# chngdickson/ov2slam

Measured on AMD Instinct MI355X. Metric: tracked_frames_per_sec, higher is better.
Workload: dtype u8/s16 fixed-point + f32

## Files before the change

include/ov2slam_hip.h:

```cpp
#ifndef OV2SLAM_HIP_H
#define OV2SLAM_HIP_H

#include <stddef.h>
#include <stdint.h>

#ifdef __cplusplus
extern "C" {
#endif

typedef int ov2_status;
enum {
    OV2_OK = 0,
    OV2_ERR_INVALID = -1,
    OV2_ERR_HIP = -2,
    OV2_ERR_NOMEM = -3,
    OV2_ERR_NODEVICE = -4,
    OV2_ERR_UNSUPPORTED = -5
};

typedef struct ov2_ctx ov2_ctx;
typedef struct ov2_images ov2_images;
typedef struct ov2_pyr ov2_pyr;

ov2_status ov2_ctx_create(int device, ov2_ctx **out);
// ... 42 lines not shown
void ov2_pyr_release(ov2_pyr *p);
void ov2_pyr_release_from(ov2_ctx *user, ov2_pyr *p);
int ov2_pyr_batch(const ov2_pyr *p);
int ov2_pyr_nlevels(const ov2_pyr *p);
ov2_status ov2_pyr_level_size(const ov2_pyr *p, int level, int *w, int *h, int *pad);
ov2_status ov2_pyr_download_level(ov2_ctx *ctx, const ov2_pyr *p, int b, int level, uint8_t *img, int16_t *grad);

ov2_status ov2_klt_track_fb(ov2_ctx *ctx, const ov2_pyr *prev, const ov2_pyr *cur, int win, int nlevels,
                            int max_iter, float eps, float err_th, float fb_th, int n, const float *kps_xy,
                            float *priors_xy, uint8_t *status);
ov2_status ov2_klt_track_fb_dev(ov2_ctx *ctx, const ov2_pyr *prev, const ov2_pyr *cur, int win, int nlevels,
                                int max_iter, float eps, float err_th, float fb_th, int n, const float *d_kps_xy,
                                float *d_priors_xy, uint8_t *d_status, const int32_t *d_img_idx,
                                uint32_t *d_iters);

ov2_status ov2_klt_tracking_frame_dev(ov2_ctx *ctx, const ov2_pyr *prev, const ov2_pyr *cur, int win,
                                      int nlevels_full, int max_iter, float eps, float err_th, float fb_th, int n,
                                      const float *d_kps_xy, const float *d_prior_xy, const uint8_t *d_has_prior,
                                      const int32_t *d_img_idx, float *d_out_xy, uint8_t *d_out_status,
                                      int32_t *d_p3p_req , uint32_t *d_iters );

ov2_status ov2_klt_set_lanes(ov2_ctx *ctx, int lanes);
ov2_status ov2_klt_set_stereo_split(ov2_ctx *ctx, int k);

ov2_status ov2_line_min_sad(ov2_ctx *ctx, const ov2_pyr *left, const ov2_pyr *right, int level, int nwinsize, int go_left,
                            int n, const float *pts_xy, float *xprior, float *l1err);
ov2_status ov2_line_min_sad_dev(ov2_ctx *ctx, const ov2_pyr *left, const ov2_pyr *right, int level, int nwinsize,
                                int go_left, int n, const float *d_pts_xy, const int32_t *d_img_idx, float *d_xprior,
                                float *d_l1err);

typedef struct ov2_cam_model {
    double K[4];
    int32_t model;
    int32_t n_coeffs;
    double D[5];
} ov2_cam_model;

ov2_status ov2_stereo_matching(ov2_ctx *ctx, const ov2_pyr *left, const ov2_pyr *right, int win, int nlevels_full,
                               int max_iter, float eps, float err_th, float fb_th, int n, const float *kps_xy,
                               const float *prior_xy, const uint8_t *has_prior, const float *lunpx_xy, int rectified,
                               const double *F_rl, const ov2_cam_model *right_cam, float *out_rxy, uint8_t *out_status);
ov2_status ov2_stereo_matching_dev(ov2_ctx *ctx, const ov2_pyr *left, const ov2_pyr *right, int win, int nlevels_full,
                                   int max_iter, float eps, float err_th, float fb_th, int n, const float *d_kps_xy,
                                   const float *d_prior_xy, const uint8_t *d_has_prior, const int32_t *d_img_idx,
                                   const float *d_lunpx_xy, int rectified, const double *F_rl, const ov2_cam_model *right_cam,
                                   float *d_out_rxy, uint8_t *d_out_status, uint32_t *d_iters);
// ... 414 lines not shown
```

ov2slam_amd/_lib.py:

```python
import ctypes as C
import os

_HERE = os.path.dirname(os.path.abspath(__file__))
LIB_PATH = os.environ.get("OV2SLAM_HIP_LIB") or os.path.join(_HERE, "lib", "libov2hip.so")

vp = C.c_void_p
vpp = C.POINTER(C.c_void_p)
ip = C.POINTER(C.c_int)
fp = C.POINTER(C.c_float)

SIGNATURES = {
    "ov2_ctx_create": (C.c_int, [C.c_int, vpp]),
    "ov2_ctx_create_ex": (C.c_int, [C.c_int, C.c_int, vpp]),
    "ov2_ctx_destroy": (None, [vp]),
    "ov2_last_error": (C.c_char_p, [vp]),
    "ov2_status_string": (C.c_char_p, [C.c_int]),
    "ov2_ctx_synchronize": (C.c_int, [vp]),
    "ov2_ctx_set_kf_overlap": (C.c_int, [vp, C.c_int]),
    "ov2_ctx_set_wave_prio": (C.c_int, [vp, C.c_int]),
    "ov2_ctx_get_wave_prio": (C.c_int, [vp]),
    "ov2_ctx_create_cu": (C.c_int, [C.c_int, C.c_int, C.c_int, C.c_int, vpp]),
    "ov2_ctx_get_cu_share": (C.c_int, [vp]),
    "ov2_ctx_get_cu_mask": (C.c_int, [vp, C.c_int, C.POINTER(C.c_uint32)]),
    "ov2_cu_mask_build": (C.c_int, [C.c_int, C.c_int, C.c_int, C.POINTER(C.c_uint32)]),
# ... 12 lines not shown
    "ov2_memcpy_d2h": (C.c_int, [vp, vp, vp, C.c_size_t]),
    "ov2_memcpy_d2d": (C.c_int, [vp, vp, vp, C.c_size_t]),
    "ov2_images_create": (C.c_int, [vp, C.c_int, C.c_int, C.c_int, vpp]),
    "ov2_images_upload": (C.c_int, [vp, vp, C.c_int, vp, C.c_int]),
    "ov2_images_destroy": (None, [vp]),
    "ov2_pyramid_build": (C.c_int, [vp, vp, C.c_int, C.c_int, C.c_int, C.c_int, C.c_int, C.c_int, C.c_float,
                                    C.c_int, C.c_int, vpp]),
    "ov2_pyramid_build_images": (C.c_int, [vp, vp, C.c_int, C.c_int, C.c_int, C.c_float, C.c_int, C.c_int, vpp]),
    "ov2_pyr_retain": (None, [vp]),
    "ov2_pyr_release": (None, [vp]),
    "ov2_pyr_release_from": (None, [vp, vp]),
    "ov2_pyr_batch": (C.c_int, [vp]),
    "ov2_pyr_nlevels": (C.c_int, [vp]),
    "ov2_pyr_level_size": (C.c_int, [vp, C.c_int, ip, ip, ip]),
    "ov2_pyr_download_level": (C.c_int, [vp, vp, C.c_int, C.c_int, vp, vp]),
    "ov2_klt_track_fb": (C.c_int, [vp, vp, vp, C.c_int, C.c_int, C.c_int, C.c_float, C.c_float, C.c_float,
                                   C.c_int, vp, vp, vp]),
    "ov2_klt_track_fb_dev": (C.c_int, [vp, vp, vp, C.c_int, C.c_int, C.c_int, C.c_float, C.c_float, C.c_float,
                                       C.c_int, vp, vp, vp, vp, vp]),
    "ov2_klt_tracking_frame_dev": (C.c_int, [vp, vp, vp, C.c_int, C.c_int, C.c_int, C.c_float, C.c_float,
                                             C.c_float, C.c_int, vp, vp, vp, vp, vp, vp, vp, vp]),
    "ov2_klt_set_lanes": (C.c_int, [vp, C.c_int]),
    "ov2_klt_set_stereo_split": (C.c_int, [vp, C.c_int]),
    "ov2_line_min_sad": (C.c_int, [vp, vp, vp, C.c_int, C.c_int, C.c_int, C.c_int, vp, vp, vp]),
    "ov2_line_min_sad_dev": (C.c_int, [vp, vp, vp, C.c_int, C.c_int, C.c_int, C.c_int, vp, vp, vp, vp]),
    "ov2_stereo_matching": (C.c_int, [vp, vp, vp, C.c_int, C.c_int, C.c_int, C.c_float, C.c_float, C.c_float, C.c_int,
                                      vp, vp, vp, vp, C.c_int, vp, vp, vp, vp]),
    "ov2_stereo_matching_dev": (C.c_int, [vp, vp, vp, C.c_int, C.c_int, C.c_int, C.c_float, C.c_float, C.c_float, C.c_int,
                                          vp, vp, vp, vp, vp, C.c_int, vp, vp, vp, vp, vp]),
    "ov2_detect_grid": (C.c_int, [vp, vp, C.c_int, C.c_int, C.c_int, C.POINTER(C.c_double), C.c_int, vp, vp, C.c_int, ip, vp]),
    "ov2_detect_grid_batch": (C.c_int, [vp, vp, C.c_int, C.c_int, C.POINTER(C.c_double), ip, vp, vp, C.c_int, ip, vp, C.c_int]),
    "ov2_detect_grid_batch_dev": (C.c_int, [vp, vp, C.c_int, C.c_int, vp, C.c_int, vp, vp, vp, vp, C.c_int, vp, vp, C.c_int]),
    "ov2_fast_detect_batch": (C.c_int, [vp, vp, C.c_int, C.c_int, vp, vp, C.c_int, C.c_int, vp, vp, vp, vp]),
    "ov2_fast_detect_batch_dev": (C.c_int, [vp, vp, C.c_int, C.c_int, C.c_int, vp, vp, C.c_int, C.c_int, vp, vp, vp, vp]),
    "ov2_ba_default_options": (None, [vp, C.c_float]),
    "ov2_ba_solve": (C.c_int, [vp, vp, vp, vp]),
    "ov2_ba_solve_batch": (C.c_int, [vp, C.c_int, vp, vp, vp]),
    "ov2_ba_solve_batch_dev": (C.c_int, [vp, C.c_int, vp, vp, vp]),
    "ov2_pnp_solve_batch_dev": (C.c_int, [vp, C.c_int, vp, vp, vp, vp, vp, vp, C.c_int, C.c_float, C.c_int, C.c_int,
                                          vp, vp, vp, vp]),
    "ov2_map_create": (C.c_int, [vp, C.c_int, C.c_int, C.c_int, vp]),
    "ov2_map_destroy": (None, [vp]),
    "ov2_map_add_keyframe": (C.c_int, [vp, C.c_int, vp, C.c_int, vp, vp, vp, vp, vp]),
    "ov2_map_set_landmarks": (C.c_int, [vp, C.c_int, vp, vp, vp]),
    "ov2_map_set_poses": (C.c_int, [vp, C.c_int, vp, vp]),
    "ov2_map_remove_obs": (C.c_int, [vp, C.c_int, vp, vp]),
# ... 87 lines not shown
```

ov2slam_amd/csrc/ctx.hip:

```cpp
#include "ov2_internal.h"

#include <cstdlib>

ov2_status ov2_set_err(ov2_ctx *ctx, ov2_status s, const char *fmt, ...)
{
    char buf[512];
    va_list ap;
    va_start(ap, fmt);
    vsnprintf(buf, sizeof(buf), fmt, ap);
    va_end(ap);
    if (ctx) {
        std::lock_guard<std::mutex> g(ctx->mu);
        ctx->err = buf;
    }
    return s;
}

extern "C" const char *ov2_status_string(ov2_status s)
{
    switch (s) {
    case OV2_OK: return "ok";
    case OV2_ERR_INVALID: return "invalid argument";
    case OV2_ERR_HIP: return "HIP runtime error";
    case OV2_ERR_NOMEM: return "out of memory";
// ... 91 lines not shown
    if (device < 0 || device >= ndev) return OV2_ERR_INVALID;
    if (hipSetDevice(device) != hipSuccess) return OV2_ERR_HIP;
    uint32_t mask[MAX_MASK_WORDS];
    int mask_words = 0, effective_cus = 0;
    if (n_cus > 0) {
        const int total = device_cus(device);
        if (n_cus >= total || total > 32 * MAX_MASK_WORDS || ov2_cu_mask_build(total, n_cus, layout, mask) != OV2_OK) return OV2_ERR_INVALID;
        mask_words = (total + 31) / 32;
        for (int x = 0; x < OV2_CU_MASK_XCDS; ++x) {
            int bits = 0, own = 0;
            for (int k = x; k < total; k += OV2_CU_MASK_XCDS, ++own) bits += (int)(mask[k >> 5] >> (k & 31) & 1u);
            effective_cus += bits ? bits : own;
        }
    }
    ov2_ctx *c = new ov2_ctx();
    c->device = device;
    c->scratch_dev = nullptr;
    c->scratch_bytes = 0;
    c->tmp_img = nullptr;
    c->ktime_on = false;
    c->wave_prio = high_priority ? OV2_WAVE_PRIO_HIGH : 0;
    c->klt_lanes = 0;
    c->klt_stereo_split = -1;
    c->knn_lanes = 0;
    c->knn_cus = effective_cus;
    c->cu_share = n_cus;
    c->cu_layout = layout;
    c->counts_as_high = false;
    c->lcd_splits = 0;
    c->lcd_calls = 0;
    c->ba_arena = nullptr;
    c->ba_arena_cap = 0;
    c->ba_host = nullptr;
    c->ba_host_cap = 0;
    c->ba_copy_stream = nullptr;
    c->klt_counts[0] = c->klt_counts[1] = nullptr;
    c->klt_counts_words = 0;
    c->klt_counts_cur = 0;
    c->klt_counts_dirty = true;
    c->ba_copy_ev[0] = c->ba_copy_ev[1] = nullptr;
    c->ba_arena2 = nullptr;
    c->ba_arena2_cap = 0;
    c->stage_host = c->stage_dev = nullptr;
    c->stage_cap = 0;
    c->stage_ev = nullptr;
    c->stage_ev_pending = false;
// ... 455 lines not shown
```

ov2slam_amd/csrc/klt.hip:

```cpp
#include <cstdlib>

#include "ov2_internal.h"
#include "ov2_wave.h"

using namespace ov2wave;

namespace {

struct klt_params {
    int win, nlevels, max_iter;
    int wave_prio;
    double eps2;
    float err_th;
    double fb_th;
    float min_eig_thr;
    int rule33;
};

#define W_BITS 14

__device__ __forceinline__ void lk_weights(float a, float b, int &w00, int &w01, int &w10, int &w11)
{
    w00 = (int)__builtin_rintf((1.f - a) * (1.f - b) * (float)(1 << W_BITS));
    w01 = (int)__builtin_rintf(a * (1.f - b) * (float)(1 << W_BITS));
// ... 403 lines not shown
    const unsigned o = J.img_o + (unsigned)(rr0 * J.istride + cc0);
#pragma unroll
    for (int t = 0; t < klt3::NLD; ++t) {
        unsigned a;
        if (klt3::RBYTES == 48) a = o + (unsigned)(t * J.istride + 16 * c);
        else {
            const int sg = min(3 * t + c, 2 * klt3::RROWS - 1);
            a = o + (unsigned)((sg >> 1) * J.istride + (sg & 1) * 16);
        }
        S.v[t] = ld_b128(J.base + (size_t)a);
    }
}
__device__ __forceinline__ void klt3_store_region(const klt3_segs &S, int c, bool store, unsigned char *lj)
{
    if (store) {
#pragma unroll
        for (int t = 0; t < klt3::NLD; ++t) {
            if (klt3::RBYTES == 48) *reinterpret_cast<uint4 *>(lj + t * klt3::RBYTES + 16 * c) = S.v[t];
            else if (3 * t + c < 2 * klt3::RROWS) *reinterpret_cast<uint4 *>(lj + (3 * t + c) * 16) = S.v[t];
        }
    }
}

template <int WIN>
__device__ __forceinline__ int lk_level3(const level_ptrs &I, const level_ptrs &J, int pad, int level, int max_level,
                                         bool run, float kx, float ky, float &nx_io, float &ny_io, int &status,
                                         float &err, const klt_params &P, int c, bool lane_ok, unsigned &passes,
                                         unsigned char *lj)
{
    static_assert(WIN == 9, "three lanes x three columns");
    constexpr int NPX = 3 * WIN, NQ = (NPX + 1) / 2;
    const float FLT_SCALE = 1.f / (float)(1 << 20);
    const float half = (float)(WIN - 1) * 0.5f;
    const float lscale = __builtin_ldexpf(1.f, -level);
    float px = kx * lscale, py = ky * lscale;
    float nx, ny;
    if (level == max_level) { nx = nx_io * lscale; ny = ny_io * lscale; }
    else { nx = nx_io * 2.f; ny = ny_io * 2.f; }
    if (run) { nx_io = nx; ny_io = ny; }

    px -= half; py -= half;
    const int ipx = (int)floorf(px), ipy = (int)floorf(py);
    if (run && (ipx < -WIN || ipx >= I.w || ipy < -WIN || ipy >= I.h)) {
        if (level == 0) { status = 0; err = 0.f; }
        run = false;
    }
    if (!__any(run)) return 0;
    if (run) passes += 1u;
    int w00, w01, w10, w11;
    lk_weights(px - (float)ipx, py - (float)ipy, w00, w01, w10, w11);

// ... 170 lines not shown
            }
        }
        float b1, b2;
        if (__all((unsigned)(pb1 + (1 << 27)) < (1u << 28) && (unsigned)(pb2 + (1 << 27)) < (1u << 28))) {
            b1 = (float)sum3_i32(pb1, c) * FLT_SCALE;
            b2 = (float)sum3_i32(pb2, c) * FLT_SCALE;
        } else {
            b1 = (float)sum3_f64((double)pb1, c) * FLT_SCALE;
            b2 = (float)sum3_f64((double)pb2, c) * FLT_SCALE;
        }
        const float dx = (A12 * b2 - A22 * b1) * D;
        const float dy = (A12 * b1 - A11 * b2) * D;
        if (run) {
            ++iters;
            nx += dx; ny += dy;
            nx_io = nx + half; ny_io = ny + half;
            if ((double)dx * dx + (double)dy * dy <= P.eps2) run = false;
            else if (j > 0 && fabsf(dx + pdx) <= 0.01f && fabsf(dy + pdy) <= 0.01f) {
                nx_io -= dx * 0.5f; ny_io -= dy * 0.5f;
                run = false;
            }
            pdx = dx; pdy = dy;
        }
    }
    return iters;
}

template <int WIN, int GL>
__device__ __forceinline__ int lk_pass(const level_ptrs &I, const level_ptrs &J, int pad, int level, int max_level, bool run,
                                       float kx, float ky, float &nx_io, float &ny_io, int &status, float &err,
                                       const klt_params &P, int sub, bool lane_ok, unsigned &passes, unsigned char *smem, int slot)
{
    if constexpr (GL == 3) {
        return lk_level3<WIN>(I, J, pad, level, max_level, run, kx, ky, nx_io, ny_io, status, err, P, sub, lane_ok, passes,
                              smem + slot * klt3::RSZ);
    } else {
        constexpr int KPW = 64 / GL, WB = klt_lds<WIN>::WB, GB = klt_lds<WIN>::GB;
        return lk_level<WIN, GL>(I, J, pad, level, max_level, run, kx, ky, nx_io, ny_io, status, err, P, sub, passes,
                                 smem + slot * WB, smem + KPW * WB + slot * WB, smem + 2 * KPW * WB + slot * GB);
    }
}

struct __attribute__((aligned(16))) klt_handover { float fx, fy, err; unsigned work; };

template <int WIN, int GL>
__device__ __forceinline__ int fb_track(const ov2_pyr_view &pv, const ov2_pyr_view &cv, int b, bool act, float kx,
                                          float ky, float &fx, float &fy, const klt_params &P, int nlevels, int sub,
                                          bool lane_ok, unsigned &work, unsigned char *smem, int slot,
                                          int l_hi, int l_lo, float err0, unsigned work0, float &err_out)
{
    int status = 1;
    float err = err0;
    unsigned it = work0 & 0xffffu, passes = work0 >> 16;
    for (int l = l_hi; l >= l_lo; --l) {
        const level_ptrs I = level_of(pv, l, b), J = level_of(cv, l, b);
        it += lk_pass<WIN, GL>(I, J, pv.pad, l, nlevels, act, kx, ky, fx, fy, status, err, P, sub, lane_ok, passes, smem, slot);
    }
    if (l_lo > 0) {
        work = it | (passes << 16);
        err_out = err;
        return 0;
    }
    const int W0 = cv.lv[0].w, H0 = cv.lv[0].h;
    int ok = act && status && !(err > P.err_th) &&
             (1.f <= fx && fx < (float)W0 - 1.f && 1.f <= fy && fy < (float)H0 - 1.f);
    int st2 = 1;
    float e2 = 0.f, bx = kx, by = ky;
    {
        const level_ptrs I = level_of(cv, 0, b), J = level_of(pv, 0, b);
        it += lk_pass<WIN, GL>(I, J, cv.pad, 0, 0, ok != 0, fx, fy, bx, by, st2, e2, P, sub, lane_ok, passes, smem, slot);
    }
    if (ok) {
        if (!st2) ok = 0;
        else {
            const float dx = kx - bx, dy = ky - by;
            const double nrm = __dsqrt_rn((double)dx * dx + (double)dy * dy);
            if (nrm > P.fb_th) ok = 0;
        }
    }
    work = it | (passes << 16);
    return ok;
}

template <int WIN, int GL>
__device__ __forceinline__ int fb_track(const ov2_pyr_view &pv, const ov2_pyr_view &cv, int b, bool act, float kx,
                                          float ky, float &fx, float &fy, const klt_params &P, int nlevels, int sub,
                                          bool lane_ok, unsigned &work, unsigned char *smem, int slot)
{
    float err;
    return fb_track<WIN, GL>(pv, cv, b, act, kx, ky, fx, fy, P, nlevels, sub, lane_ok, work, smem, slot, nlevels, 0, 0.f, 0u, err);
}

#define KLT_GL8_MIN_KPS 65536
// ... 101 lines not shown
    const bool retry = mine && is_a && !ok;
    const unsigned long long rm = __ballot(retry);
    if (rm) {
        const int lane = (int)threadIdx.x, leader = __ffsll((long long)rm) - 1;
        int base = 0;
        if (lane == leader) base = (int)atomicAdd(&cnt[2], (unsigned)__popcll(rm));
        base = __shfl(base, leader);
        if (retry) list_c[base + __popcll(rm & ((1ull << lane) - 1ull))] = i;
    }
}

template <int WIN, int KLT_GL, bool SPLIT>
__global__ __launch_bounds__(64) __attribute__((amdgpu_waves_per_eu(KLT_WAVES(WIN, KLT_GL)))) void klt_stage1_kernel(ov2_pyr_view pv, ov2_pyr_view cv, klt_params P, int n,
                                                        const float2 *__restrict__ kps,
                                                        const float2 *__restrict__ prior,
                                                        const int *__restrict__ img_idx, float2 *__restrict__ out_xy,
                                                        unsigned char *__restrict__ out_status,
                                                        unsigned *__restrict__ counts ,
                                                        unsigned *__restrict__ iters, const int *__restrict__ list_a,
                                                        const int *__restrict__ list_b, unsigned *__restrict__ cnt,
                                                        int *__restrict__ list_c,
                                                        int b_word ,
                                                        int split_k ,
                                                        klt_handover *__restrict__ hand )
{
    __shared__ __attribute__((aligned(16))) unsigned char smem[klt_smem<WIN, KLT_GL>::BYTES];
    using M = klt_map<KLT_GL>;
    constexpr int KLT_KPW = M::KPW;
    const int total_a = (int)cnt[0], total_b = (int)cnt[b_word];
    const int groups_b = (total_b + KLT_KPW - 1) / KLT_KPW;
    const bool is_a = (int)blockIdx.x >= groups_b;
    const int g = is_a ? (int)blockIdx.x - groups_b : (int)blockIdx.x;
    const int total = is_a ? total_a : total_b;
    if (g * KLT_KPW >= total) return;
    ov2wave::set_wave_prio(P.wave_prio);
    const int slot = M::slot((int)threadIdx.x), sub = M::sub((int)threadIdx.x), idx = g * KLT_KPW + slot;
    const bool lane_ok = M::lane_ok((int)threadIdx.x);
    const bool act = idx < total && lane_ok;
    const int i = (is_a ? list_a : list_b)[idx < total ? idx : total - 1];
    const float2 kp = kps[i];
    const int b = img_idx ? img_idx[i] : 0;
    float2 pr = (is_a || !P.rule33) ? prior[i] : kp;
    unsigned work = 0;
    const int nl = is_a ? min(1, pv.nlevels - 1) : P.nlevels;
    const bool upper = SPLIT && !is_a;
    float err;
    const int ok = fb_track<WIN, KLT_GL>(pv, cv, b, act, kp.x, kp.y, pr.x, pr.y, P, nl, sub, lane_ok, work, smem, slot, nl,
                                         upper ? split_k + 1 : 0, 0.f, 0u, err);
    if (upper) {
        if (act && sub == 0) hand[i] = klt_handover{pr.x, pr.y, err, work};
        return;
    }
    klt_stage1_finish(act && sub == 0, is_a, i, b, n, ok, pr, work, out_xy, out_status, counts, iters, cnt, list_c);
}

template <int WIN, int KLT_GL>
__global__ __launch_bounds__(64) __attribute__((amdgpu_waves_per_eu(KLT_WAVES(WIN, KLT_GL)))) void klt_stage2_kernel(ov2_pyr_view pv, ov2_pyr_view cv, klt_params P, int n,
                                                        const float2 *__restrict__ kps,
                                                        const int *__restrict__ img_idx, float2 *__restrict__ out_xy,
                                                        unsigned char *__restrict__ out_status,
                                                        const unsigned *__restrict__ counts, int *__restrict__ p3p_req,
                                                        unsigned *__restrict__ iters, const int *__restrict__ list_c,
                                                        const unsigned *__restrict__ cnt, int batch,
                                                        unsigned *__restrict__ next_counts, int next_words,
                                                        const int *__restrict__ list_b, int b_word,
                                                        const float2 *__restrict__ prior,
                                                        int split_k ,
                                                        const klt_handover *__restrict__ hand)
{
    __shared__ __attribute__((aligned(16))) unsigned char smem[klt_smem<WIN, KLT_GL>::BYTES];
    using M = klt_map<KLT_GL>;
    constexpr int KLT_KPW = M::KPW;
    const int slot = M::slot((int)threadIdx.x), sub = M::sub((int)threadIdx.x);
    const bool lane_ok = M::lane_ok((int)threadIdx.x);
    for (int q = blockIdx.x * 64 + threadIdx.x; q < next_words; q += gridDim.x * 64) next_counts[q] = 0u;
    auto tally = [&](int b, int &n3, int &good) {
        n3 = 0; good = 0;
        if constexpr (KLT_GL == 3) {
            for (int q = sub; q < 64; q += 3) {
                const unsigned cw = counts[64 * b + q];
                n3 += (int)(cw & 0xffffu); good += (int)(cw >> 16);
            }
            n3 = sum3_i32(n3, sub); good = sum3_i32(good, sub);
        } else {
            for (int q = 0; q < 64 / KLT_GL; ++q) {
                const unsigned cw = counts[64 * b + sub * (64 / KLT_GL) + q];
                n3 += (int)(cw & 0xffffu); good += (int)(cw >> 16);
            }
            n3 = row_sum_i32<KLT_GL>(n3); good = row_sum_i32<KLT_GL>(good);
        }
    };
// ... 19 lines not shown
    const int i = (is_b ? list_b : list_c)[idx < total ? idx : total - 1];
    const int b = img_idx ? img_idx[i] : 0;
    const float2 kp = kps[i];
    float2 pr;
    int l_hi = P.nlevels;
    float err0 = 0.f;
    unsigned work0 = 0;
    if (is_b) {
        if (split_k >= 0) {
            const klt_handover hr = hand[i];
            pr = make_float2(hr.fx, hr.fy);
            err0 = hr.err; work0 = hr.work; l_hi = split_k;
        } else {
            pr = prior[i];
        }
    } else {
        int n3, good;
        tally(b, n3, good);
        const bool drop = P.rule33 && n3 > 0 && (double)good < 0.33 * (double)n3;
        pr = drop ? kp : out_xy[i];
    }
    unsigned work = 0;
    float err;
    const int ok = fb_track<WIN, KLT_GL>(pv, cv, b, act, kp.x, kp.y, pr.x, pr.y, P, P.nlevels, sub, lane_ok, work, smem, slot,
                                         l_hi, 0, err0, work0, err);
    if (act && sub == 0) {
        out_xy[i] = pr;
        out_status[i] = (unsigned char)ok;
        if (iters) iters[n + i] = work;
    }
}

int klt_lanes_for(const ov2_ctx *c, int n, int win, const ov2_pyr *a, const ov2_pyr *b)
{
    static const int env = [] { const char *e = getenv("OV2_KLT_LANES"); return e ? atoi(e) : 0; }();
    const int forced = c->klt_lanes ? c->klt_lanes : env;
    const bool fits32 = a->buf->bytes < (1ull << 32) && b->buf->bytes < (1ull << 32);
    if (forced == 8 || forced == 16 || (forced == 3 && win == 9 && fits32)) return forced;
    if (win == 9 && fits32) return 3;
    return n >= KLT_GL8_MIN_KPS ? 8 : 16;
}

ov2_status make_params(ov2_ctx *c, const ov2_pyr *prev, const ov2_pyr *cur, int win, int nlevels, int max_iter,
                       float eps, float err_th, float fb_th, klt_params *P)
{
    if (!prev || !cur) return ov2_set_err(c, OV2_ERR_INVALID, "null pyramid");
    const ov2_pyr_view &a = prev->buf->view, &b = cur->buf->view;
    if (a.nlevels != b.nlevels || a.pad != b.pad || a.batch != b.batch || a.lv[0].w != b.lv[0].w ||
// ... 5 lines not shown
    if (a.nlevels < nlevels + 1) nlevels = a.nlevels - 1;
    P->win = win;
    P->wave_prio = c->wave_prio;
    P->nlevels = nlevels;
    P->max_iter = max_iter < 0 ? 0 : (max_iter > 100 ? 100 : max_iter);
    double e = (double)eps;
    if (e < 0.) e = 0.;
    if (e > 10.) e = 10.;
    P->eps2 = e * e;
    P->err_th = err_th;
    P->fb_th = (double)fb_th;
    P->min_eig_thr = 1e-4f;
    P->rule33 = 1;
    return OV2_OK;
}

}

extern "C" ov2_status ov2_klt_set_lanes(ov2_ctx *c, int lanes)
{
    if (!c) return OV2_ERR_INVALID;
    if (lanes != 0 && lanes != 3 && lanes != 8 && lanes != 16) return ov2_set_err(c, OV2_ERR_INVALID, "lanes per keypoint: 0 (auto), 3, 8 or 16");
    c->klt_lanes = lanes;
    return OV2_OK;
}

extern "C" ov2_status ov2_klt_set_stereo_split(ov2_ctx *c, int k)
{
    if (!c) return OV2_ERR_INVALID;
    c->klt_stereo_split = k < 0 ? -1 : k;
    return OV2_OK;
}

extern "C" ov2_status ov2_klt_track_fb_dev(ov2_ctx *c, const ov2_pyr *prev, const ov2_pyr *cur, int win, int nlevels,
                                           int max_iter, float eps, float err_th, float fb_th, int n,
                                           const float *d_kps, float *d_priors, uint8_t *d_status,
                                           const int32_t *d_img_idx, uint32_t *d_iters)
{
    if (!c) return OV2_ERR_INVALID;
    if (n == 0) return OV2_OK;
    if (n < 0 || !d_kps || !d_priors || !d_status) return ov2_set_err(c, OV2_ERR_INVALID, "null/negative argument");
    klt_params P;
    ov2_status s = make_params(c, prev, cur, win, nlevels, max_iter, eps, err_th, fb_th, &P);
    if (s != OV2_OK) return s;
    OV2_HIP(c, hipSetDevice(c->device));
    if ((s = ov2_pyr_wait_ready(c, prev)) != OV2_OK || (s = ov2_pyr_wait_ready(c, cur)) != OV2_OK) return s;
// ... 99 lines not shown
    unsigned *counts = c->klt_counts[c->klt_counts_cur], *live_cnt = counts + (size_t)B * 64;
    unsigned *next_counts = c->klt_counts[c->klt_counts_cur ^ 1];
    const int next_words = (int)c->klt_counts_words;
    int *list_a = (int *)scr, *list_b = list_a + n, *list_c = list_b + n;
    if (c->kf.want_stereo_ev) {
        OV2_HIP(c, hipEventRecord(c->kf.fork, c->stream.h));
        c->kf.want_stereo_ev = false;
    }
    const dim3 cgrid((n + KLT_COMPACT_KPWG - 1) / KLT_COMPACT_KPWG);
    const int want_k = c->klt_stereo_split < 0 ? KLT_STEREO_SPLIT_DEFAULT : c->klt_stereo_split;
    const int split_k = (!P.rule33 && want_k < P.nlevels) ? want_k : -1;
    const int b_word1 = (P.rule33 || split_k >= 0) ? 1 : 3, b_word2 = P.rule33 ? 3 : 1;
    klt_handover *hand = reinterpret_cast<klt_handover *>((char *)scr + lists_bytes);
#define KLT_STAGES_GL(W, G)                                                                                     \
    do {                                                                                                        \
         \
        const dim3 tgrid((n + klt_map<G>::KPW - 1) / klt_map<G>::KPW + 2);                                      \
        OV2_LAUNCH(c, OV2_K_DETECT + 4, klt_compact_kernel, cgrid, dim3(256), 0, c->stream, n, d_has_prior,     \
                   d_iters, list_a, list_b, live_cnt, d_p3p_req, B, P.wave_prio);                               \
        if (split_k >= 0)                                                                                       \
            OV2_LAUNCH(c, OV2_K_KLT_STAGE1, (klt_stage1_kernel<W, G, true>), tgrid, dim3(64), 0, c->stream,     \
                       prev->buf->view, cur->buf->view, P, n, reinterpret_cast<const float2 *>(d_kps),          \
                       reinterpret_cast<const float2 *>(d_prior), d_img_idx, reinterpret_cast<float2 *>(d_out_xy), \
                       d_out_status, counts, d_iters, list_a, list_b, live_cnt, list_c, b_word1, split_k, hand); \
        else                                                                                                    \
            OV2_LAUNCH(c, OV2_K_KLT_STAGE1, (klt_stage1_kernel<W, G, false>), tgrid, dim3(64), 0, c->stream,    \
                       prev->buf->view, cur->buf->view, P, n, reinterpret_cast<const float2 *>(d_kps),          \
                       reinterpret_cast<const float2 *>(d_prior), d_img_idx, reinterpret_cast<float2 *>(d_out_xy), \
                       d_out_status, counts, d_iters, list_a, list_b, live_cnt, list_c, b_word1, split_k, hand); \
        OV2_LAUNCH(c, OV2_K_KLT_STAGE2, (klt_stage2_kernel<W, G>), tgrid, dim3(64), 0, c->stream,               \
                   prev->buf->view, cur->buf->view, P, n, reinterpret_cast<const float2 *>(d_kps), d_img_idx,   \
                   reinterpret_cast<float2 *>(d_out_xy), d_out_status, counts, d_p3p_req, d_iters, list_c,      \
                   live_cnt, B, next_counts, next_words, list_b, b_word2,                                       \
                   reinterpret_cast<const float2 *>(d_prior), split_k, hand);                                   \
    } while (0)
#define KLT_STAGES(W)                                                                                           \
    do {                                                                                                        \
        if (lanes == 8) KLT_STAGES_GL(W, 8);                                                                       \
        else KLT_STAGES_GL(W, 16);                                                                              \
    } while (0)
    switch (win) {
    case 3: KLT_STAGES(3); break;
    case 5: KLT_STAGES(5); break;
    case 7: KLT_STAGES(7); break;
    case 9:
        if (lanes == 3) KLT_STAGES_GL(9, 3);
        else KLT_STAGES(9);
        break;
    default: KLT_STAGES(11); break;
    }
#undef KLT_STAGES
#undef KLT_STAGES_GL
    OV2_HIP(c, hipGetLastError());
    c->klt_counts_cur ^= 1;
    c->klt_counts_dirty = false;
    return OV2_OK;
}
// ... 1 lines not shown
```

ov2slam_amd/csrc/ov2_internal.h:

```cpp
#pragma once
#include <hip/hip_runtime.h>

#include <atomic>
#include <cstdarg>
#include <cstdio>
#include <cstring>
#include <mutex>
#include <string>
#include <vector>

#include "../../include/ov2slam_hip.h"

#define OV2_MAX_LEVELS 8
#define OV2_LM 16

struct ov2_level_desc {
    int w, h;
    int istride;
    int gstride;
    int rows;
    size_t img_off;
    size_t grad_off;
    size_t img_bstride;
    size_t grad_bstride;
// ... 76 lines not shown
    std::string err;
    void *scratch_dev;
    size_t scratch_bytes;
    ov2_images *tmp_img;
    void *ba_arena;
    size_t ba_arena_cap;
    void *stage_host, *stage_dev;
    size_t stage_cap;
    hipEvent_t stage_ev;
    bool stage_ev_pending;
    void *ba_arena2;
    size_t ba_arena2_cap;
    void *ba_host;
    size_t ba_host_cap;
    unsigned *klt_counts[2];
    size_t klt_counts_words;
    int klt_counts_cur;
    bool klt_counts_dirty;
    hipStream_t ba_copy_stream;
    hipEvent_t ba_copy_ev[2];
    int wave_prio;
    int klt_lanes;
    int klt_stereo_split;
    int knn_lanes;
    int knn_cus;
    int cu_share, cu_layout;
    bool counts_as_high;
    int lcd_splits;
    long long lcd_calls;
    std::vector<struct ov2_lcd_table *> lcd_tables;
    bool ktime_on;
    std::vector<ov2_ktime_rec> ktime_recs;
    std::vector<hipEvent_t> ktime_free;
};

struct ov2_images {
    ov2_ctx *ctx;
    int batch, w, h;
    int stride;
    size_t bstride;
    unsigned char *base;
};

struct ov2_pyr {
    std::atomic<int> refs;
    ov2_ctx *ctx;
// ... 42 lines not shown
```

ov2slam_amd/frontend.py:

```python
import ctypes as C

import numpy as np

from . import _lib


WAVE_PRIO_HIGH = 2


CU_LAYOUT_SPREAD, CU_LAYOUT_PACKED = 0, 1
CU_MASK_XCDS = 8


def cu_mask_build(total_cus, n_cus, layout=CU_LAYOUT_SPREAD):
    out = (C.c_uint32 * ((int(total_cus) + 31) // 32 if total_cus > 0 else 1))()
    st = _lib.load().ov2_cu_mask_build(int(total_cus), int(n_cus), int(layout), out)
    if st != 0:
        raise _lib.Ov2Error(f"ov2_cu_mask_build({total_cus}, {n_cus}, {layout}): status {st}")
    return np.array(out, np.uint32)


def _check(ctx_handle, status):
    if status != 0:
        lib = _lib.load()
# ... 11 lines not shown
        else:
            st = self.lib.ov2_ctx_create_cu(device, int(bool(high_priority)), int(cu_share), int(cu_layout), C.byref(h))
            if st == -1:
                raise _lib.Ov2Error(f"ov2_ctx_create_cu(device={device}, high_priority={bool(high_priority)}, n_cus={cu_share}, "
                                    f"layout={cu_layout}): {self.lib.ov2_status_string(st).decode()}")
        if st != 0:
            raise _lib.Ov2Error(f"ov2_ctx_create(device={device}): {self.lib.ov2_status_string(st).decode()} -- "
                                "an MI355X/gfx950 device is required, there is no CPU fallback")
        self.h = h

    def close(self):
        if getattr(self, "h", None):
            self.lib.ov2_ctx_destroy(self.h)
            self.h = None

    def __del__(self):
        self.close()

    def set_klt_lanes(self, lanes):
        _check(self.h, self.lib.ov2_klt_set_lanes(self.h, int(lanes)))

    def set_stereo_split(self, k):
        _check(self.h, self.lib.ov2_klt_set_stereo_split(self.h, int(k)))

    def set_knn_lanes(self, lanes):
        _check(self.h, self.lib.ov2_knn_set_lanes(self.h, int(lanes)))

    def set_kf_overlap(self, on):
        _check(self.h, self.lib.ov2_ctx_set_kf_overlap(self.h, int(bool(on))))

    def set_wave_prio(self, level):
        _check(self.h, self.lib.ov2_ctx_set_wave_prio(self.h, int(level)))

    def get_wave_prio(self):
        return int(self.lib.ov2_ctx_get_wave_prio(self.h))

    def get_cu_share(self):
        return int(self.lib.ov2_ctx_get_cu_share(self.h))

    def get_cu_mask(self, words):
        out = (C.c_uint32 * int(words))()
        _check(self.h, self.lib.ov2_ctx_get_cu_mask(self.h, int(words), out))
        return np.array(out, np.uint32)

    def set_pyr_ring(self, n):
        _check(self.h, self.lib.ov2_ctx_set_pyr_ring(self.h, int(n)))
# ... 345 lines not shown
```

Before: 293,700.

## Repack straggler KLT keypoints into wide wavefront tail for 3-lane tracker

Measured after the change: 292,600. About the same (-0.4%).

```diff
diff --git a/include/ov2slam_hip.h b/include/ov2slam_hip.h
--- a/include/ov2slam_hip.h
+++ b/include/ov2slam_hip.h
@@ -88,6 +88,7 @@
 
 ov2_status ov2_klt_set_lanes(ov2_ctx *ctx, int lanes);
 ov2_status ov2_klt_set_stereo_split(ov2_ctx *ctx, int k);
+ov2_status ov2_klt_set_wide_stats(ov2_ctx *ctx, uint32_t *d_words);
 
 ov2_status ov2_line_min_sad(ov2_ctx *ctx, const ov2_pyr *left, const ov2_pyr *right, int level, int nwinsize, int go_left,
                             int n, const float *pts_xy, float *xprior, float *l1err);
diff --git a/ov2slam_amd/_lib.py b/ov2slam_amd/_lib.py
--- a/ov2slam_amd/_lib.py
+++ b/ov2slam_amd/_lib.py
@@ -58,6 +58,7 @@
                                              C.c_float, C.c_int, vp, vp, vp, vp, vp, vp, vp, vp]),
     "ov2_klt_set_lanes": (C.c_int, [vp, C.c_int]),
     "ov2_klt_set_stereo_split": (C.c_int, [vp, C.c_int]),
+    "ov2_klt_set_wide_stats": (C.c_int, [vp, vp]),
     "ov2_line_min_sad": (C.c_int, [vp, vp, vp, C.c_int, C.c_int, C.c_int, C.c_int, vp, vp, vp]),
     "ov2_line_min_sad_dev": (C.c_int, [vp, vp, vp, C.c_int, C.c_int, C.c_int, C.c_int, vp, vp, vp, vp]),
     "ov2_stereo_matching": (C.c_int, [vp, vp, vp, C.c_int, C.c_int, C.c_int, C.c_float, C.c_float, C.c_float, C.c_int,
diff --git a/ov2slam_amd/csrc/ctx.hip b/ov2slam_amd/csrc/ctx.hip
--- a/ov2slam_amd/csrc/ctx.hip
+++ b/ov2slam_amd/csrc/ctx.hip
@@ -137,6 +137,7 @@
     c->wave_prio = high_priority ? OV2_WAVE_PRIO_HIGH : 0;
     c->klt_lanes = 0;
     c->klt_stereo_split = -1;
+    c->klt_wide_stats = nullptr;
     c->knn_lanes = 0;
     c->knn_cus = effective_cus;
     c->cu_share = n_cus;
diff --git a/ov2slam_amd/csrc/klt.hip b/ov2slam_amd/csrc/klt.hip
--- a/ov2slam_amd/csrc/klt.hip
+++ b/ov2slam_amd/csrc/klt.hip
@@ -449,11 +449,165 @@
     }
 }
 
+#ifndef KLT3_WIDE_J0
+#define KLT3_WIDE_J0 2
+#endif
+#define KLT3_WIDE_MAX_KPS 2
+#ifndef KLT3_WIDE_PLAIN
+#define KLT3_WIDE_PLAIN 0
+#endif
+#define KLT3_WIDE_TPL_STRIDE 176
+
+__device__ __forceinline__ float klt3_bcast(float v, int l0, int l1, bool h)
+{
+    const int a = __builtin_amdgcn_readlane(__float_as_int(v), l0), b = __builtin_amdgcn_readlane(__float_as_int(v), l1);
+    return __int_as_float(h ? b : a);
+}
+__device__ __forceinline__ int klt3_bcast(int v, int l0, int l1, bool h)
+{
+    const int a = __builtin_amdgcn_readlane(v, l0), b = __builtin_amdgcn_readlane(v, l1);
+    return h ? b : a;
+}
+__device__ __forceinline__ float klt3_half_sum(int v, bool h)
+{
+    const int s = row_sum_i32<16>(v);
+    const int a0 = __builtin_amdgcn_readlane(s, 0), a1 = __builtin_amdgcn_readlane(s, 16);
+    const int a2 = __builtin_amdgcn_readlane(s, 32), a3 = __builtin_amdgcn_readlane(s, 48);
+    return (float)((double)(h ? a2 : a0) + (double)(h ? a3 : a1));
+}
+
 template <int WIN>
+__device__ __forceinline__ void klt3_wide_tail(const level_ptrs &J, int pad, int level, const klt_params &P,
+                                            unsigned long long rmask ,
+                                            int j0 , bool run, int c, float A11, float A12, float A22,
+                                            float D, float nx, float ny, float pdx, float pdy, int rr0, int cc0,
+                                            const unsigned (&Iv2)[(3 * WIN + 1) / 2], const unsigned (&Ix2)[(3 * WIN + 1) / 2],
+                                            const unsigned (&Iy2)[(3 * WIN + 1) / 2], float &nx_io, float &ny_io, int &status,
+                                            int &iters, unsigned char *smem0, unsigned *wstats)
+{
+    constexpr int NQ = (3 * WIN + 1) / 2;
+    static_assert(3 * NQ * 4 <= KLT3_WIDE_TPL_STRIDE && 3 * KLT3_WIDE_TPL_STRIDE <= klt3::RSZ, "a template fits a region block");
+    const float FLT_SCALE = 1.f / (float)(1 << 20);
+    const float half = (float)(WIN - 1) * 0.5f;
+    const int tid = (int)threadIdx.x, t = tid & 31;
+    const bool h = tid >= 32;
+    const int l0 = __ffsll((long long)rmask) - 1;
+    const unsigned long long rest = rmask & ~(7ull << l0);
+    const bool two = rest != 0ull;
+    const int l1 = two ? __ffsll((long long)rest) - 1 : l0;
+    const int g0 = (l0 * 171) >> 9, g1 = (l1 * 171) >> 9;
+    int f0 = 0;
+    while (f0 == g0 || f0 == g1) ++f0;
+    int f1 = f0 + 1;
+    while (f1 == g0 || f1 == g1) ++f1;
+    if (run) {
+        uint4 *dst = reinterpret_cast<uint4 *>(smem0 + (tid - c == l0 ? f0 : f1) * klt3::RSZ + c * KLT3_WIDE_TPL_STRIDE);
+        unsigned tp[3 * NQ + 2];
+#pragma unroll
+        for (int q = 0; q < NQ; ++q) { tp[q] = Iv2[q]; tp[NQ + q] = Ix2[q]; tp[2 * NQ + q] = Iy2[q]; }
+        tp[3 * NQ] = tp[3 * NQ + 1] = 0u;
+#pragma unroll
+        for (int q = 0; q < (3 * NQ + 2) / 4; ++q) dst[q] = make_uint4(tp[4 * q], tp[4 * q + 1], tp[4 * q + 2], tp[4 * q + 3]);
+    }
+    bool wrun = !h || two;
+    A11 = klt3_bcast(A11, l0, l1, h); A12 = klt3_bcast(A12, l0, l1, h); A22 = klt3_bcast(A22, l0, l1, h);
+    D = klt3_bcast(D, l0, l1, h);
+    nx = klt3_bcast(nx, l0, l1, h); ny = klt3_bcast(ny, l0, l1, h);
+    pdx = klt3_bcast(pdx, l0, l1, h); pdy = klt3_bcast(pdy, l0, l1, h);
+    rr0 = klt3_bcast(rr0, l0, l1, h); cc0 = klt3_bcast(cc0, l0, l1, h);
+    const unsigned img_o = (unsigned)klt3_bcast((int)J.img_o, l0, l1, h);
+    float wx_io = klt3_bcast(nx_io, l0, l1, h), wy_io = klt3_bcast(ny_io, l0, l1, h);
+    int wstatus = klt3_bcast(status, l0, l1, h), wit = klt3_bcast(iters, l0, l1, h);
+    unsigned char *lj = smem0 + (h ? g1 : g0) * klt3::RSZ;
+    __syncthreads();
+    const bool px_ok = wrun && t < WIN * 3;
+    const int r = px_ok ? (t * 171) >> 9 : 0, cw = px_ok ? t - 3 * r : 0;
+    unsigned V01, V2, X01, X2, Y01, Y2;
+    {
+        const unsigned short *tp = reinterpret_cast<const unsigned short *>(smem0 + (h ? f1 : f0) * klt3::RSZ + cw * KLT3_WIDE_TPL_STRIDE) + 3 * r;
+        const unsigned m = px_ok ? 0xffffffffu : 0u;
+        V01 = ((unsigned)tp[0] | ((unsigned)tp[1] << 16)) & m; V2 = (unsigned)tp[2] & m;
+        X01 = ((unsigned)tp[2 * NQ] | ((unsigned)tp[2 * NQ + 1] << 16)) & m; X2 = (unsigned)tp[2 * NQ + 2] & m;
+        Y01 = ((unsigned)tp[4 * NQ] | ((unsigned)tp[4 * NQ + 1] << 16)) & m; Y2 = (unsigned)tp[4 * NQ + 2] & m;
+    }
+    unsigned trips = 0;
+    for (int j = j0; j < P.max_iter; ++j) {
+        if (!__any(wrun)) break;
+        ++trips;
+        const int inx = (int)floorf(nx), iny = (int)floorf(ny);
+        if (wrun && (inx < -WIN || inx >= J.w || iny < -WIN || iny >= J.h)) {
+            if (level == 0) wstatus = 0;
+            wrun = false;
+        }
+        int w00j, w01j, w10j, w11j;
+        lk_weights(nx - (float)inx, ny - (float)iny, w00j, w01j, w10j, w11j);
+        int rb = wrun ? iny + pad - rr0 : 0, cb = wrun ? OV2_LM + inx - cc0 : 0;
+        const bool out = (unsigned)rb > (unsigned)klt3::ROW_SPAN || (unsigned)cb > (unsigned)klt3::COL_SPAN;
+        if (__any(out)) {
+            static_assert(klt3::RBYTES == 48 && 3 * klt3::RROWS <= 64, "two pieces per lane of a half");
+            __syncthreads();
+            if (out) {
+                klt3_region_origin(J, pad, inx, iny, rr0, cc0);
+                const unsigned o = img_o + (unsigned)(rr0 * J.istride + cc0);
+                const int p1 = min(t + 32, 3 * klt3::RROWS - 1);
+                const int ra = (t * 171) >> 9, rb1 = (p1 * 171) >> 9;
+                const uint4 sa = ld_b128(J.base + (size_t)(o + (unsigned)(ra * J.istride + 16 * (t - 3 * ra))));
+                const uint4 sb = ld_b128(J.base + (size_t)(o + (unsigned)(rb1 * J.istride + 16 * (p1 - 3 * rb1))));
+                *reinterpret_cast<uint4 *>(lj + 16 * t) = sa;
+                *reinterpret_cast<uint4 *>(lj + 16 * p1) = sb;
+                rb = iny + pad - rr0; cb = OV2_LM + inx - cc0;
+            }
+            __syncthreads();
+        }
+        const unsigned W01 = pack_lo16((unsigned)w00j, (unsigned)w01j), W23 = pack_lo16((unsigned)w10j, (unsigned)w11j);
+        const int cq = cb + 3 * cw;
+        const unsigned *q = reinterpret_cast<const unsigned *>(lj + (rb + r) * klt3::RBYTES + (cq & ~3));
+        const unsigned *qr = q + klt3::RBYTES / 4;
+        unsigned a[3];
+#pragma unroll
+        for (int i = 0; i < 3; ++i) {
+            const unsigned sel = klt3_pair_sel(((unsigned)cq & 3u) + (unsigned)i);
+            const unsigned T = __builtin_amdgcn_perm(q[1], q[0], sel), B = __builtin_amdgcn_perm(qr[1], qr[0], sel);
+            a[i] = (unsigned)dot2(B, W23, dot2k(T, W01, 1 << (W_BITS - 5 - 1)));
+        }
+        const unsigned d01 = pk_sub16(shr_pack_hi<W_BITS - 5>(a[0] >> (W_BITS - 5), a[1]), V01);
+        const unsigned d2 = pk_sub16(a[2] >> (W_BITS - 5), V2);
+        const int pb1 = dot2(d2, X2, dot2(d01, X01, 0)), pb2 = dot2(d2, Y2, dot2(d01, Y01, 0));
+        const float b1 = klt3_half_sum(pb1, h) * FLT_SCALE, b2 = klt3_half_sum(pb2, h) * FLT_SCALE;
+        const float dx = (A12 * b2 - A22 * b1) * D;
+        const float dy = (A12 * b1 - A11 * b2) * D;
+        if (wrun) {
+            ++wit;
+            nx += dx; ny += dy;
+            wx_io = nx + half; wy_io = ny + half;
+            if ((double)dx * dx + (double)dy * dy <= P.eps2) wrun = false;
+            else if (j > 0 && fabsf(dx + pdx) <= 0.01f && fabsf(dy + pdy) <= 0.01f) {
+                wx_io -= dx * 0.5f; wy_io -= dy * 0.5f;
+                wrun = false;
+            }
+            pdx = dx; pdy = dy;
+        }
+    }
+    const float x0 = __int_as_float(__builtin_amdgcn_readlane(__float_as_int(wx_io), 0)), x1 = __int_as_float(__builtin_amdgcn_readlane(__float_as_int(wx_io), 32));
+    const float y0 = __int_as_float(__builtin_amdgcn_readlane(__float_as_int(wy_io), 0)), y1 = __int_as_float(__builtin_amdgcn_readlane(__float_as_int(wy_io), 32));
+    const int s0 = __builtin_amdgcn_readlane(wstatus, 0), s1 = __builtin_amdgcn_readlane(wstatus, 32);
+    const int i0 = __builtin_amdgcn_readlane(wit, 0), i1 = __builtin_amdgcn_readlane(wit, 32);
+    if (run) {
+        const bool first = tid - c == l0;
+        nx_io = first ? x0 : x1; ny_io = first ? y0 : y1;
+        status = first ? s0 : s1; iters = first ? i0 : i1;
+    }
+    if (wstats) {
+        if (tid == 0) { atomicAdd(&wstats[0], 1u); atomicAdd(&wstats[1], trips); }
+    }
+}
+
+template <int WIN, bool WIDE>
 __device__ __forceinline__ int lk_level3(const level_ptrs &I, const level_ptrs &J, int pad, int level, int max_level,
                                          bool run, float kx, float ky, float &nx_io, float &ny_io, int &status,
                                          float &err, const klt_params &P, int c, bool lane_ok, unsigned &passes,
-                                         unsigned char *lj)
+                                         unsigned char *lj, unsigned char *smem0 ,
+                                         unsigned *wstats )
 {
     static_assert(WIN == 9, "three lanes x three columns");
     constexpr int NPX = 3 * WIN, NQ = (NPX + 1) / 2;
@@ -670,18 +824,27 @@
             }
             pdx = dx; pdy = dy;
         }
+        if constexpr (WIDE) {
+            const unsigned long long rmask = __ballot(run);
+            if (rmask != 0ull && __popcll(rmask) <= 3 * KLT3_WIDE_MAX_KPS && j + 1 >= KLT3_WIDE_J0 && j + 1 < P.max_iter) {
+                klt3_wide_tail<WIN>(J, pad, level, P, rmask, j + 1, run, c, A11, A12, A22, D, nx, ny, pdx, pdy, rr0, cc0, Iv2, Ix2,
+                                    Iy2, nx_io, ny_io, status, iters, smem0, wstats);
+                return iters;
+            }
+        }
     }
     return iters;
 }
 
-template <int WIN, int GL>
+template <int WIN, int GL, bool WIDE>
 __device__ __forceinline__ int lk_pass(const level_ptrs &I, const level_ptrs &J, int pad, int level, int max_level, bool run,
                                        float kx, float ky, float &nx_io, float &ny_io, int &status, float &err,
-                                       const klt_params &P, int sub, bool lane_ok, unsigned &passes, unsigned char *smem, int slot)
+                                       const klt_params &P, int sub, bool lane_ok, unsigned &passes, unsigned char *smem, int slot,
+                                       unsigned *wstats)
 {
     if constexpr (GL == 3) {
-        return lk_level3<WIN>(I, J, pad, level, max_level, run, kx, ky, nx_io, ny_io, status, err, P, sub, lane_ok, passes,
-                              smem + slot * klt3::RSZ);
+        return lk_level3<WIN, WIDE>(I, J, pad, level, max_level, run, kx, ky, nx_io, ny_io, status, err, P, sub, lane_ok, passes,
+                                    smem + slot * klt3::RSZ, smem, wstats);
     } else {
         constexpr int KPW = 64 / GL, WB = klt_lds<WIN>::WB, GB = klt_lds<WIN>::GB;
         return lk_level<WIN, GL>(I, J, pad, level, max_level, run, kx, ky, nx_io, ny_io, status, err, P, sub, passes,
@@ -691,18 +854,19 @@
 
 struct __attribute__((aligned(16))) klt_handover { float fx, fy, err; unsigned work; };
 
-template <int WIN, int GL>
+template <int WIN, int GL, bool WIDE = false>
 __device__ __forceinline__ int fb_track(const ov2_pyr_view &pv, const ov2_pyr_view &cv, int b, bool act, float kx,
                                           float ky, float &fx, float &fy, const klt_params &P, int nlevels, int sub,
                                           bool lane_ok, unsigned &work, unsigned char *smem, int slot,
-                                          int l_hi, int l_lo, float err0, unsigned work0, float &err_out)
+                                          int l_hi, int l_lo, float err0, unsigned work0, float &err_out,
+                                          unsigned *wstats = nullptr )
 {
     int status = 1;
     float err = err0;
     unsigned it = work0 & 0xffffu, passes = work0 >> 16;
     for (int l = l_hi; l >= l_lo; --l) {
         const level_ptrs I = level_of(pv, l, b), J = level_of(cv, l, b);
-        it += lk_pass<WIN, GL>(I, J, pv.pad, l, nlevels, act, kx, ky, fx, fy, status, err, P, sub, lane_ok, passes, smem, slot);
+        it += lk_pass<WIN, GL, WIDE>(I, J, pv.pad, l, nlevels, act, kx, ky, fx, fy, status, err, P, sub, lane_ok, passes, smem, slot, wstats);
     }
     if (l_lo > 0) {
         work = it | (passes << 16);
@@ -716,7 +880,7 @@
     float e2 = 0.f, bx = kx, by = ky;
     {
         const level_ptrs I = level_of(cv, 0, b), J = level_of(pv, 0, b);
-        it += lk_pass<WIN, GL>(I, J, cv.pad, 0, 0, ok != 0, fx, fy, bx, by, st2, e2, P, sub, lane_ok, passes, smem, slot);
+        it += lk_pass<WIN, GL, WIDE>(I, J, cv.pad, 0, 0, ok != 0, fx, fy, bx, by, st2, e2, P, sub, lane_ok, passes, smem, slot, wstats);
     }
     if (ok) {
         if (!st2) ok = 0;
@@ -864,7 +1028,8 @@
                                                         int *__restrict__ list_c,
                                                         int b_word ,
                                                         int split_k ,
-                                                        klt_handover *__restrict__ hand )
+                                                        klt_handover *__restrict__ hand ,
+                                                        unsigned *__restrict__ wide_stats )
 {
     __shared__ __attribute__((aligned(16))) unsigned char smem[klt_smem<WIN, KLT_GL>::BYTES];
     using M = klt_map<KLT_GL>;
@@ -887,8 +1052,9 @@
     const int nl = is_a ? min(1, pv.nlevels - 1) : P.nlevels;
     const bool upper = SPLIT && !is_a;
     float err;
-    const int ok = fb_track<WIN, KLT_GL>(pv, cv, b, act, kp.x, kp.y, pr.x, pr.y, P, nl, sub, lane_ok, work, smem, slot, nl,
-                                         upper ? split_k + 1 : 0, 0.f, 0u, err);
+    constexpr bool WIDE = KLT_GL == 3 && (SPLIT || KLT3_WIDE_PLAIN);
+    const int ok = fb_track<WIN, KLT_GL, WIDE>(pv, cv, b, act, kp.x, kp.y, pr.x, pr.y, P, nl, sub, lane_ok, work, smem, slot, nl,
+                                               upper ? split_k + 1 : 0, 0.f, 0u, err, wide_stats);
     if (upper) {
         if (act && sub == 0) hand[i] = klt_handover{pr.x, pr.y, err, work};
         return;
@@ -908,7 +1074,8 @@
                                                         const int *__restrict__ list_b, int b_word,
                                                         const float2 *__restrict__ prior,
                                                         int split_k ,
-                                                        const klt_handover *__restrict__ hand)
+                                                        const klt_handover *__restrict__ hand,
+                                                        unsigned *__restrict__ wide_stats )
 {
     __shared__ __attribute__((aligned(16))) unsigned char smem[klt_smem<WIN, KLT_GL>::BYTES];
     using M = klt_map<KLT_GL>;
@@ -974,8 +1141,8 @@
     }
     unsigned work = 0;
     float err;
-    const int ok = fb_track<WIN, KLT_GL>(pv, cv, b, act, kp.x, kp.y, pr.x, pr.y, P, P.nlevels, sub, lane_ok, work, smem, slot,
-                                         l_hi, 0, err0, work0, err);
+    const int ok = fb_track<WIN, KLT_GL, KLT_GL == 3>(pv, cv, b, act, kp.x, kp.y, pr.x, pr.y, P, P.nlevels, sub, lane_ok, work, smem, slot,
+                                                      l_hi, 0, err0, work0, err, wide_stats);
     if (act && sub == 0) {
         out_xy[i] = pr;
         out_status[i] = (unsigned char)ok;
@@ -1027,6 +1194,13 @@
     if (!c) return OV2_ERR_INVALID;
     if (lanes != 0 && lanes != 3 && lanes != 8 && lanes != 16) return ov2_set_err(c, OV2_ERR_INVALID, "lanes per keypoint: 0 (auto), 3, 8 or 16");
     c->klt_lanes = lanes;
+    return OV2_OK;
+}
+
+extern "C" ov2_status ov2_klt_set_wide_stats(ov2_ctx *c, uint32_t *d_words)
+{
+    if (!c) return OV2_ERR_INVALID;
+    c->klt_wide_stats = d_words;
     return OV2_OK;
 }
 
@@ -1172,17 +1346,17 @@
             OV2_LAUNCH(c, OV2_K_KLT_STAGE1, (klt_stage1_kernel<W, G, true>), tgrid, dim3(64), 0, c->stream,     \
                        prev->buf->view, cur->buf->view, P, n, reinterpret_cast<const float2 *>(d_kps),          \
                        reinterpret_cast<const float2 *>(d_prior), d_img_idx, reinterpret_cast<float2 *>(d_out_xy), \
-                       d_out_status, counts, d_iters, list_a, list_b, live_cnt, list_c, b_word1, split_k, hand); \
+                       d_out_status, counts, d_iters, list_a, list_b, live_cnt, list_c, b_word1, split_k, hand, c->klt_wide_stats); \
         else                                                                                                    \
             OV2_LAUNCH(c, OV2_K_KLT_STAGE1, (klt_stage1_kernel<W, G, false>), tgrid, dim3(64), 0, c->stream,    \
                        prev->buf->view, cur->buf->view, P, n, reinterpret_cast<const float2 *>(d_kps),          \
                        reinterpret_cast<const float2 *>(d_prior), d_img_idx, reinterpret_cast<float2 *>(d_out_xy), \
-                       d_out_status, counts, d_iters, list_a, list_b, live_cnt, list_c, b_word1, split_k, hand); \
+                       d_out_status, counts, d_iters, list_a, list_b, live_cnt, list_c, b_word1, split_k, hand, c->klt_wide_stats); \
         OV2_LAUNCH(c, OV2_K_KLT_STAGE2, (klt_stage2_kernel<W, G>), tgrid, dim3(64), 0, c->stream,               \
                    prev->buf->view, cur->buf->view, P, n, reinterpret_cast<const float2 *>(d_kps), d_img_idx,   \
                    reinterpret_cast<float2 *>(d_out_xy), d_out_status, counts, d_p3p_req, d_iters, list_c,      \
                    live_cnt, B, next_counts, next_words, list_b, b_word2,                                       \
-                   reinterpret_cast<const float2 *>(d_prior), split_k, hand);                                   \
+                   reinterpret_cast<const float2 *>(d_prior), split_k, hand, c->klt_wide_stats);                \
     } while (0)
 #define KLT_STAGES(W)                                                                                           \
     do {                                                                                                        \
diff --git a/ov2slam_amd/csrc/ov2_internal.h b/ov2slam_amd/csrc/ov2_internal.h
--- a/ov2slam_amd/csrc/ov2_internal.h
+++ b/ov2slam_amd/csrc/ov2_internal.h
@@ -122,6 +122,7 @@
     int wave_prio;
     int klt_lanes;
     int klt_stereo_split;
+    unsigned *klt_wide_stats;
     int knn_lanes;
     int knn_cus;
     int cu_share, cu_layout;
diff --git a/ov2slam_amd/frontend.py b/ov2slam_amd/frontend.py
--- a/ov2slam_amd/frontend.py
+++ b/ov2slam_amd/frontend.py
@@ -57,6 +57,9 @@
 
     def set_stereo_split(self, k):
         _check(self.h, self.lib.ov2_klt_set_stereo_split(self.h, int(k)))
+
+    def set_klt_wide_stats(self, d_words):
+        _check(self.h, self.lib.ov2_klt_set_wide_stats(self.h, None if d_words is None else d_words.ptr))
 
     def set_knn_lanes(self, lanes):
         _check(self.h, self.lib.ov2_knn_set_lanes(self.h, int(lanes)))
```
